# marcopesavento/Super-resolution-3D-Human-Shape-from-a-Single-Low-Resolution-Image

Hardware: AMD Instinct MI355X
Metric: occupancy queries/sec (dense 512^3 reconstruction: encoder + query sweep + 2x marching cubes) (higher is better)
Workload: dtype bf16

## Files before the change

super-resolution-3d-human-shape-from-a-single-low-resolution-image_amd/csrc/surs_api.cpp:

```cpp
#include "surs_common.h"

extern "C" int surs_abi_version(void) { return SURS_ABI_VERSION; }

extern "C" const char *surs_last_error(void) { return surs::err_buf(); }

extern "C" int surs_device_info(int *cu_count, char *arch_out) {
    int dev = 0;
    SURS_HIP_CHECK(hipGetDevice(&dev));
    hipDeviceProp_t prop;
    SURS_HIP_CHECK(hipGetDeviceProperties(&prop, dev));
    if (cu_count) *cu_count = prop.multiProcessorCount;
    if (arch_out) {
        strncpy(arch_out, prop.gcnArchName, 31);
        arch_out[31] = 0;
    }
    return 0;
}

#include <atomic>
#include <cstdlib>
#include <mutex>

namespace {
struct OptionRow {
    const char *name, *env;
    int def;
    char env_first;
    int env_value;
    const char *what;
};
const OptionRow kOptions[surs::OPT_COUNT] = {
    {"split_parts", "SURS_SPLIT", 2, 'b', 3, "operand parts of the fp32-grade GEMMs: 2 (f16 x 2) or 3 (bf16 x 3; env: bf16x3)"},
    {"grid_f32_columns", "SURS_GRID_F32", 1, 'g', 0, "0 (env: gemm): the fp32 sweep on the per-point layer kernels"},
    {"grid_kernel", "SURS_GRID_KERNEL", 0, 0, 0, "reduced-precision column kernel: 0 (default 12), 3, 10, 12"},
    {"grid_f32_kernel", "SURS_GRID_F32_KERNEL", 0, 0, 0, "fp32-grade column kernel: 0 (default 11), 5, 11"},
    {"r_parts", "SURS_R_PARTS", 1, 0, 0, "1: the bf16 sweep's R vectors from one f16 part; 0: the sweep's split"},
    {"grid_f32_passes", "SURS_GRID_F32_PASSES", 2, 0, 0, "passes of the fp32-grade column kernel per batch: 2 (lr, then hr) or 1"},
    {"bicubic_block", "SURS_BICUBIC_BLOCK", 1, 0, 0, "0: bicubic x2 with statistics one output per item (A/B; same bits)"},
    {"mc_emit_reclassify", "SURS_MC_EMIT_RECLASSIFY", 0, 0, 0, "1: marching cubes' emit pass classifies again (tests)"},
    {"point_runs_speculate", "SURS_POINT_RUNS_SPECULATE", 1, 0, 0, "0: surs_query_points_columns reads the run count before it launches"},
    {"conv_trace", "SURS_CONV_TRACE", 0, 0, 0, "diagnostic builds (-DSURS_CONV_TRACE): print the 3x3 kernel's phase stamps"},
    {"v3_trace", "SURS_V3_TRACE", 0, 0, 0, "diagnostic builds (-DSURS_V3_TRACE): print the column kernels' stamps"},
    {"conv_tall_min_wg", "SURS_CONV_TALL_MIN_WG", 256, 0, 0, "workgroups from which a stride-1 3x3 convolution takes the 8-row tile instead of 4 rows (0: never; same bits)"},
    {"conv_wide_min_wg", "SURS_CONV_WIDE_MIN_WG", 512, 0, 0, "workgroups (of 64 channels) from which such a launch takes 8 rows x 64 channels (part of the bits: another order of sums; 0: never)"},
    {"mc_ring", "SURS_MC_RING", 258, 0, 0, "planes of marching cubes' edge -> vertex-id ring = layers per chunk of a one-piece extraction + 1 (66: round 5's)"},
    {"rvec_small", "SURS_RVEC_SMALL", 1, 0, 0, "0: the affine part's GEMM of batches of <= 1024 columns on the 256 x 256-tile kernel (A/B; same bits)"},
};
std::atomic<int> g_option[surs::OPT_COUNT];
std::once_flag g_option_once;
void import_environment() {
    for (int i = 0; i < surs::OPT_COUNT; ++i) {
        const OptionRow &r = kOptions[i];
        int v = r.def;
        if (const char *e = getenv(r.env)) {
            if (r.env_first) v = (e[0] == r.env_first) ? r.env_value : r.def;
            else if (e[0]) v = atoi(e);
        }
        g_option[i].store(v, std::memory_order_relaxed);
    }
}
int find_option(const char *name) {
    if (!name) return -1;
    for (int i = 0; i < surs::OPT_COUNT; ++i)
        if (!strcmp(name, kOptions[i].name) || !strcmp(name, kOptions[i].env)) return i;
    return -1;
}
}

int surs::option(surs::Opt id) {
    std::call_once(g_option_once, import_environment);
    return g_option[id].load(std::memory_order_relaxed);
}

extern "C" int surs_set_option(const char *name, int value) {
    const int i = find_option(name);
    SURS_REQUIRE(i >= 0, "unknown option '%s' (surs_option_name(i) lists them)", name ? name : "(null)");
    std::call_once(g_option_once, import_environment);
    g_option[i].store(value, std::memory_order_relaxed);
    return 0;
}

extern "C" int surs_get_option(const char *name, int *value) {
    const int i = find_option(name);
    SURS_REQUIRE(i >= 0 && value, "unknown option '%s'", name ? name : "(null)");
    *value = surs::option((surs::Opt)i);
    return 0;
}

extern "C" const char *surs_option_name(int index) { return (index >= 0 && index < surs::OPT_COUNT) ? kOptions[index].name : nullptr; }
extern "C" const char *surs_option_help(int index) { return (index >= 0 && index < surs::OPT_COUNT) ? kOptions[index].what : nullptr; }
```

super-resolution-3d-human-shape-from-a-single-low-resolution-image_amd/csrc/surs_common.h:

```cpp
#pragma once
#include <hip/hip_runtime.h>

#include <cstdarg>
#include <cstdio>
#include <cstring>

#include "../../include/surs.h"

namespace surs {

inline char *err_buf() {
    static thread_local char buf[512] = "";
    return buf;
}

inline int fail(int code, const char *fmt, ...) {
    va_list ap;
    va_start(ap, fmt);
    vsnprintf(err_buf(), 512, fmt, ap);
    va_end(ap);
    return code;
}

#define SURS_HIP_CHECK(expr)                                                                     \
    do {                                                                                         \
        hipError_t e_ = (expr);                                                                  \
        if (e_ != hipSuccess)                                                                    \
            return surs::fail(SURS_E_HIP, "%s:%d %s -> %s", __FILE__, __LINE__, #expr, hipGetErrorString(e_)); \
    } while (0)

#define SURS_LAUNCH_CHECK() SURS_HIP_CHECK(hipGetLastError())

#define SURS_REQUIRE(cond, ...)                                   \
    do {                                                          \
        if (!(cond)) return surs::fail(SURS_E_INVALID, __VA_ARGS__); \
    } while (0)

#ifndef SURS_ABL_NO_ISA_PINS
#define SURS_ISA_PIN(v) asm volatile("" : "+v"(v))
#else
#define SURS_ISA_PIN(v) do { } while (0)
#endif

enum Opt {
    OPT_SPLIT_PARTS, OPT_GRID_F32_COLUMNS, OPT_GRID_KERNEL, OPT_GRID_F32_KERNEL, OPT_R_PARTS,
    OPT_GRID_F32_PASSES, OPT_BICUBIC_BLOCK, OPT_MC_EMIT_RECLASSIFY, OPT_POINT_RUNS_SPECULATE, OPT_CONV_TRACE,
    OPT_V3_TRACE, OPT_CONV_TALL_MIN_WG, OPT_CONV_WIDE_MIN_WG, OPT_MC_RING, OPT_RVEC_SMALL, OPT_COUNT
};
int option(Opt id);

inline hipStream_t as_stream(void *s) { return reinterpret_cast<hipStream_t>(s); }

constexpr int ceil_div(long long a, long long b) { return (int)((a + b - 1) / b); }

struct DeviceOnce {
    unsigned long long mask = 0;
    bool first() {
        int dev = 0;
        if (hipGetDevice(&dev) != hipSuccess || dev < 0 || dev >= 64) return true;
        const unsigned long long bit = 1ull << dev;
        const unsigned long long old = __atomic_fetch_or(&mask, bit, __ATOMIC_ACQ_REL);
        return !(old & bit);
    }
};
inline size_t align_up(size_t v, size_t a) { return (v + a - 1) / a * a; }

}
```

super-resolution-3d-human-shape-from-a-single-low-resolution-image_amd/csrc/surs_gemm.inc:

```
__device__ __forceinline__ bool gemm_block_tile(int mblocks, int nblocks, int &mb, int &nb) {
    const unsigned total = (unsigned)mblocks * (unsigned)nblocks, per = gridDim.x >> 3;
    const unsigned logical = (blockIdx.x & 7u) * per + (blockIdx.x >> 3);
    mb = (int)(logical % (unsigned)mblocks);
    nb = (int)(logical / (unsigned)mblocks);
    return logical < total;
}

static inline unsigned gemm_grid(int mblocks, long long nblocks) {
    const long long total = (long long)mblocks * nblocks;
    return (unsigned)(((total + 7) / 8) * 8);
}

struct SplitSeg {
    const unsigned short *base;
    long long part;
    int ktiles;
};

constexpr int G3_STAGES = 3;
constexpr int g3_stage_bytes(int bm, int np_ = 3) { return np_ * ((bm / 32) + 8) * 1024; }
constexpr int g3_lds_bytes(int bm, int np_ = 3) { return G3_STAGES * g3_stage_bytes(bm, np_); }

template <int NP> struct SplitKind;
template <> struct SplitKind<1> {
// ... 263 lines not shown
    const unsigned short *xp = a.g[m] + ((size_t)n0 + li) * 16 + kh * 8;
    const long long g_part = a.g_part[m];
    f32x16 acc[2];
#pragma unroll
    for (int j = 0; j < 2; ++j)
#pragma unroll
        for (int q = 0; q < 16; ++q) acc[j][q] = 0.0f;
    vec8 wf[PF][NP], xf[PF][2][NP];
    auto fetch = [&](int kt, int s) {
#pragma unroll
        for (int p = 0; p < NP; ++p) {
            wf[s][p] = *reinterpret_cast<const vec8 *>(wp + (size_t)kt * D2 * 16 + p * w_part);
#pragma unroll
            for (int j = 0; j < 2; ++j) xf[s][j][p] = *reinterpret_cast<const vec8 *>(xp + ((size_t)kt * npm + 32 * j) * 16 + p * g_part);
        }
    };
#pragma unroll
    for (int s = 0; s < PF; ++s) fetch(s, s);
    for (int k0 = 0; k0 < KT; k0 += PF) {
#pragma unroll
        for (int s = 0; s < PF; ++s) {
            vec8 w_[NP], x_[2][NP];
#pragma unroll
            for (int p = 0; p < NP; ++p) {
                w_[p] = wf[s][p];
                x_[0][p] = xf[s][0][p];
                x_[1][p] = xf[s][1][p];
            }
            if (k0 + PF + s < KT) fetch(k0 + PF + s, s);
#pragma unroll
            for (int t = 0; t < NP; ++t)
#pragma unroll
                for (int j = 0; j < 2; ++j) acc[j] = SK::mfma(x_[j][t], w_[NP - 1 - t], acc[j]);
            if (NP == 3) {
#pragma unroll
                for (int j = 0; j < 2; ++j) acc[j] = SK::mfma(x_[j][0], w_[1], acc[j]);
#pragma unroll
                for (int j = 0; j < 2; ++j) acc[j] = SK::mfma(x_[j][1], w_[0], acc[j]);
            }
            if (NP >= 2) {
#pragma unroll
                for (int j = 0; j < 2; ++j) acc[j] = SK::mfma(x_[j][0], w_[0], acc[j]);
            }
        }
    }
    float *out = a.r[m];
#pragma unroll
    for (int j = 0; j < 2; ++j)
#pragma unroll
        for (int gq = 0; gq < 4; ++gq)
#pragma unroll
            for (int r = 0; r < 4; ++r) out[(n0 + 32 * j + 4 * kh + 8 * gq + r) * D2 + m0 + li] = acc[j][4 * gq + r] + 0.0f;
}
```

super-resolution-3d-human-shape-from-a-single-low-resolution-image_amd/csrc/surs_query.hip:

```cpp
#include <hip/hip_runtime.h>

#include <cstdlib>
#include <map>
#include <mutex>
#include <type_traits>
#include <utility>
#include <vector>

#include "surs_common.h"
#include "surs_mlp_generic.h"
#include "surs_mlp_layout.h"

namespace surs {

typedef float f32x16 __attribute__((ext_vector_type(16)));
typedef float f32x4 __attribute__((ext_vector_type(4)));
typedef unsigned u32x4 __attribute__((ext_vector_type(4)));
typedef unsigned u32x2 __attribute__((ext_vector_type(2)));
typedef float f32x2 __attribute__((ext_vector_type(2)));

struct PointSource {
    int mode;
    const float *pts;
    const long long *idx;
// ... 66 lines not shown
    pix[1] = (long long)cy0 * W + cx1;
    pix[2] = (long long)cy1 * W + cx0;
    pix[3] = (long long)cy1 * W + cx1;
}

__device__ __forceinline__ float tap_sum(const float (&t)[4], const float (&w)[4]) {
    float a = 0.0f;
    a += t[0] * w[0];
    a += t[1] * w[1];
    a += t[2] * w[2];
    a += t[3] * w[3];
    return a;
}

typedef __bf16 bf16x8_t __attribute__((ext_vector_type(8)));
typedef unsigned short u16x8_t __attribute__((ext_vector_type(8)));

__device__ __forceinline__ void split3_bf16(float x, unsigned short &a, unsigned short &b, unsigned short &c) {
    const __bf16 ha = (__bf16)x;
    const float r1 = x - (float)ha;
    const __bf16 hb = (__bf16)r1;
    const float r2 = r1 - (float)hb;
    const __bf16 hc = (__bf16)r2;
    a = __builtin_bit_cast(unsigned short, ha);
    b = __builtin_bit_cast(unsigned short, hb);
    c = __builtin_bit_cast(unsigned short, hc);
}

#include "surs_gemm.inc"

template <int NP>
__global__ __launch_bounds__(256) void gather_kernel(PointSource src, long long n, const float *__restrict__ feat_lr,
                                                     int hl, int wl, const float *__restrict__ feat_hr, int hh,
                                                     int wh, float *__restrict__ F, long long ldf,
                                                     float *__restrict__ mask, float *__restrict__ zproj,
                                                     unsigned short *__restrict__ Fs, long long fs_part) {
    __shared__ float tile[64][65];
    __shared__ float sx[64], sy[64];
    const int tid = threadIdx.x, lane = tid & 63, wave = tid >> 6;
    const long long n0 = (long long)blockIdx.x * 64;
    const bool lead = blockIdx.y == 0;
    if (tid < 64) {
        long long t = n0 + tid;
        float X = 2.0f, Y = 2.0f;
        if (t < n) {
            float px, py, pz;
            make_point(src, t, px, py, pz);
            float Z;
            project_point(src, px, py, pz, X, Y, Z);
            const float in = in_image(X, Y);
            if (lead) {
                mask[t] = in;
                if (zproj) zproj[t] = Z;
                F[(long long)C_G * ldf + t] = Z * src.zmul / src.zdiv;
                F[(long long)(C_G + 1) * ldf + t] = 0.0f;
            }
            if (Fs && lead) {
                unsigned short zp[NP];
                SplitKind<NP>::split(Z * src.zmul / src.zdiv, zp);
#pragma unroll
                for (int p = 0; p < NP; ++p) {
                    u16x8_t v = {zp[p], 0, 0, 0, 0, 0, 0, 0}, z = {0, 0, 0, 0, 0, 0, 0, 0};
                    u16x8_t *dst = reinterpret_cast<u16x8_t *>(Fs + p * fs_part + ((long long)(C_G / 16) * ldf + t) * 16);
                    dst[0] = v;
                    dst[1] = z;
                }
            }
        }
        sx[tid] = X;
        sy[tid] = Y;
    }
    __syncthreads();
    for (int chunk = blockIdx.y; chunk < 5; chunk += gridDim.y) {
        const bool is_hr = chunk == 4;
        const float *feat = is_hr ? feat_hr : feat_lr;
        const int H = is_hr ? hh : hl, W = is_hr ? wh : wl, C = is_hr ? C_HR : C_LR;
        const int c0 = is_hr ? 0 : chunk * 64;
        for (int q0 = 0; q0 < 16; q0 += 8) {
            float t[8][4], w[8][4];
#pragma unroll
            for (int u4 = 0; u4 < 8; ++u4) {
                const int p = wave * 16 + q0 + u4;
                long long pix[4];
                bilinear_taps(sx[p], sy[p], H, W, pix, w[u4]);
                const long long ch = c0 + lane;
#pragma unroll
                for (int q = 0; q < 4; ++q) t[u4][q] = feat[pix[q] * C + ch];
            }
#pragma unroll
            for (int u4 = 0; u4 < 8; ++u4) tile[lane][wave * 16 + q0 + u4] = tap_sum(t[u4], w[u4]);
        }
        __syncthreads();
        const int cbase = is_hr ? C_LR : chunk * 64;
        for (int q = 0; q < 16; ++q) {
            const int ch = wave * 16 + q;
            if (n0 + lane < n) F[(long long)(cbase + ch) * ldf + n0 + lane] = tile[ch][lane];
        }
        if (Fs) {
#pragma unroll
            for (int it = 0; it < 2; ++it) {
                const int item = tid + 256 * it, p = item & 63, half = (item >> 6) & 1, ktl = item >> 7;
                u16x8_t q[NP];
#pragma unroll
                for (int j = 0; j < 8; ++j) {
                    unsigned short parts[NP];
                    SplitKind<NP>::split(tile[ktl * 16 + half * 8 + j][p], parts);
#pragma unroll
                    for (int k = 0; k < NP; ++k) q[k][j] = parts[k];
                }
                if (n0 + p < n) {
                    unsigned short *dst = Fs + ((long long)(cbase / 16 + ktl) * ldf + n0 + p) * 16 + half * 8;
#pragma unroll
                    for (int k = 0; k < NP; ++k) *reinterpret_cast<u16x8_t *>(dst + k * fs_part) = q[k];
                }
            }
        }
        __syncthreads();
    }
}

template <int NP>
__global__ __launch_bounds__(256) void mlp_last_kernel(const float *__restrict__ w4,
                                                       const float *__restrict__ Y3, const float *__restrict__ F,
                                                       long long ld, long long n, const float *__restrict__ mask,
                                                       float *__restrict__ pred, float *__restrict__ logit,
                                                       float *__restrict__ p_slot, unsigned short *__restrict__ Fs,
                                                       long long fs_part) {
    const long long t = (long long)blockIdx.x * 256 + threadIdx.x;
    if (t >= n) return;
    float acc = w4[D4 + C0PAD];
    for (int k = 0; k < D4; ++k) acc = fmaf(w4[k], Y3[(long long)k * ld + t], acc);
    for (int k = 0; k < C_G + 2; ++k) acc = fmaf(w4[D4 + k], F[(long long)k * ld + t], acc);
    const float p = mask[t] * (1.0f / (1.0f + expf(-acc)));
    pred[t] = p;
    if (logit) logit[t] = acc;
    if (p_slot) p_slot[t] = p;
    if (Fs) {
        unsigned short parts[NP];
        SplitKind<NP>::split(p, parts);
        unsigned short *dst = Fs + ((long long)(C_G / 16) * ld + t) * 16 + 1;
#pragma unroll
        for (int k = 0; k < NP; ++k) dst[k * fs_part] = parts[k];
    }
}

template <int NP>
__global__ __launch_bounds__(256) void patch_plr_kernel(const float *__restrict__ p_lr, long long ld, long long n, float *__restrict__ p_slot,
                                                        unsigned short *__restrict__ Fs, long long fs_part) {
    const long long t = (long long)blockIdx.x * 256 + threadIdx.x;
    if (t >= n) return;
// ... 55 lines not shown
    for (int k = 0; k < C_G + 2; ++k) acc = fmaf(w4[D4 + k], Fm[(long long)k * ld + t], acc);
    const float y = 1.0f / (1.0f + expf(-acc));
    if (logit) logit[t] = acc;
    for (int v = 0; v < nviews; ++v) {
        const float p = mask[(long long)v * ld + t] * y;
        pred[(long long)v * n + t] = p;
        if (p_slot) p_slot[(long long)v * f_view_stride + t] = p;
        if (Fs) {
            unsigned short parts[NP];
            SplitKind<NP>::split(p, parts);
            unsigned short *dst = Fs + (long long)v * NP * fs_part + ((long long)(C_G / 16) * ld + t) * 16 + 1;
#pragma unroll
            for (int k = 0; k < NP; ++k) dst[k * fs_part] = parts[k];
        }
    }
}

struct Fp32Workspace {
    float *F, *Y3, *mask;
    unsigned short *Fs, *Y0s, *Y1s, *Y2s;
    long long np;
};

static size_t fp32_ws_bytes(long long np) {
    return (size_t)np * ((C0PAD + D4 + 1) * sizeof(float) + (size_t)(C0PAD + D1 + D2 + D3) * 6) + 4096;
}

static Fp32Workspace carve_fp32(void *ws, long long np) {
    Fp32Workspace w;
    float *p = (float *)ws;
    w.np = np;
    w.F = p; p += (size_t)C0PAD * np;
    w.Y3 = p; p += (size_t)D4 * np;
    w.mask = p; p += np;
    unsigned short *q = (unsigned short *)p;
    w.Fs = q; q += (size_t)3 * C0PAD * np;
    w.Y0s = q; q += (size_t)3 * D1 * np;
    w.Y1s = q; q += (size_t)3 * D2 * np;
    w.Y2s = q;
    return w;
}

static int g_split_override = 0;
static thread_local int t_split_call = 0;
static int split_parts() {
    const int v = option(OPT_SPLIT_PARTS) == 3 ? 3 : 2;
    return t_split_call > 1 ? t_split_call : (g_split_override ? g_split_override : v);
}

template <int NP, int... More, class F> static void with_parts(int parts, F &&f) {
    if constexpr (sizeof...(More) == 0) f(std::integral_constant<int, NP>());
    else if (parts == NP) f(std::integral_constant<int, NP>());
    else with_parts<More...>(parts, f);
}

static int g3_set_attributes() {
    static DeviceOnce attr;
    if (attr.first()) {
        SURS_HIP_CHECK(hipFuncSetAttribute((const void *)gemm_x3g_kernel<8, 256, G3_SPLIT, 2>, hipFuncAttributeMaxDynamicSharedMemorySize, g3_lds_bytes(256, 2)));
        SURS_HIP_CHECK(hipFuncSetAttribute((const void *)gemm_x3g_kernel<8, 256, G3_F32, 2>, hipFuncAttributeMaxDynamicSharedMemorySize, g3_lds_bytes(256, 2)));
        SURS_HIP_CHECK(hipFuncSetAttribute((const void *)gemm_x3g_kernel<8, 128, G3_F32, 2>, hipFuncAttributeMaxDynamicSharedMemorySize, g3_lds_bytes(128, 2)));
        SURS_HIP_CHECK(hipFuncSetAttribute((const void *)gemm_x3g_kernel<8, 128, G3_F32_T, 2>, hipFuncAttributeMaxDynamicSharedMemorySize, g3_lds_bytes(128, 2)));
        SURS_HIP_CHECK(hipFuncSetAttribute((const void *)gemm_x3g_kernel<8, 256, G3_SPLIT>, hipFuncAttributeMaxDynamicSharedMemorySize, g3_lds_bytes(256)));
        SURS_HIP_CHECK(hipFuncSetAttribute((const void *)gemm_x3g_kernel<8, 256, G3_F32>, hipFuncAttributeMaxDynamicSharedMemorySize, g3_lds_bytes(256)));
        SURS_HIP_CHECK(hipFuncSetAttribute((const void *)gemm_x3g_kernel<8, 128, G3_F32>, hipFuncAttributeMaxDynamicSharedMemorySize, g3_lds_bytes(128)));
        SURS_HIP_CHECK(hipFuncSetAttribute((const void *)gemm_x3g_kernel<8, 128, G3_F32_T>, hipFuncAttributeMaxDynamicSharedMemorySize, g3_lds_bytes(128)));
        SURS_HIP_CHECK(hipFuncSetAttribute((const void *)gemm_x3g_kernel<8, 256, G3_F32_T, 2>, hipFuncAttributeMaxDynamicSharedMemorySize, g3_lds_bytes(256, 2)));
        SURS_HIP_CHECK(hipFuncSetAttribute((const void *)gemm_x3g_kernel<8, 256, G3_F32_T>, hipFuncAttributeMaxDynamicSharedMemorySize, g3_lds_bytes(256)));
        SURS_HIP_CHECK(hipFuncSetAttribute((const void *)gemm_x3g_kernel<8, 256, G3_F32_T, 1>, hipFuncAttributeMaxDynamicSharedMemorySize, g3_lds_bytes(256, 1)));
        SURS_HIP_CHECK(hipFuncSetAttribute((const void *)gemm_x3g_kernel<8, 256, G3_SPLIT, 1>, hipFuncAttributeMaxDynamicSharedMemorySize, g3_lds_bytes(256, 1)));
        SURS_HIP_CHECK(hipFuncSetAttribute((const void *)gemm_x3g_kernel<8, 256, G3_F32, 1>, hipFuncAttributeMaxDynamicSharedMemorySize, g3_lds_bytes(256, 1)));
        SURS_HIP_CHECK(hipFuncSetAttribute((const void *)gemm_x3g_kernel<8, 128, G3_F32, 1>, hipFuncAttributeMaxDynamicSharedMemorySize, g3_lds_bytes(128, 1)));
    }
    return 0;
}

static int launch_layer(hipStream_t st, int parts, int out, const void *W, int M, SplitSeg s1, SplitSeg s2, long long np, long long n,
                        const float *bias, float *Y, unsigned short *Ys) {
    SURS_REQUIRE(parts >= 1 && parts <= 3, "layer kernel: 1, 2 or 3 operand parts");
    SURS_REQUIRE(np % 256 == 0 && n % 256 == 0 && n <= np, "the layer kernel needs 256-point tiles");
    SURS_REQUIRE(M % 256 == 0 || (out != G3_SPLIT && M % 128 == 0), "layer kernel rows: a multiple of 256 (of 128 for an fp32 output)");
    SURS_REQUIRE(M % 256 == 0 || out != G3_F32_T || parts > 1, "no one-part layer kernel for a transposed output of 128-row tiles");
    int rc = g3_set_attributes();
    if (rc) return rc;
    const int K = 16 * (s1.ktiles + s2.ktiles), nb = (int)(n / 256);
    const long long ldy = out == G3_F32_T ? M : np;
    with_parts<1, 2, 3>(parts, [&](auto NP) {
        auto go = [&](auto BM, auto OUT) {
            hipLaunchKernelGGL((gemm_x3g_kernel<8, BM, OUT, NP>), dim3(gemm_grid(M / BM, nb)), dim3(512), g3_lds_bytes(BM, NP), st,
                               (const unsigned short *)W, M, K, s1, s2, np, bias, Y, ldy, Ys, (long long)M * np, nb);
        };
        using C256 = std::integral_constant<int, 256>;
        using C128 = std::integral_constant<int, 128>;
        if (out == G3_SPLIT) go(C256(), std::integral_constant<int, G3_SPLIT>());
        else if (out == G3_F32) {
            if (M % 256 == 0) go(C256(), std::integral_constant<int, G3_F32>());
            else go(C128(), std::integral_constant<int, G3_F32>());
        } else if (M % 256 == 0) go(C256(), std::integral_constant<int, G3_F32_T>());
        else if constexpr (NP > 1) go(C128(), std::integral_constant<int, G3_F32_T>());
    });
    SURS_LAUNCH_CHECK();
    return 0;
}

static int run_points_fp32(hipStream_t st, const PointSource &src, long long n, const float *feat_lr, int hl, int wl,
                           const float *feat_hr, int hh, int wh, const char *blob, const MlpBlobHeader &h,
// ... 58 lines not shown
    const float *colmask;
    const float *zvec;
    const char *core;
    const char *corex;
    const char *b1frag;
    const char *w1t;
    const char *w1tx;
    const float *rvec_lr, *rvec_hr;
    long long rld_lr, rld_hr;
    float zmid;
    unsigned *colctr;
    int phase;
    unsigned long long *kstat;
    float b1_inv_scale;
    float *vol_hr, *vol_lr;
    int ncols, rz;
    int zstride;
    const int *kcount;
    const unsigned short *klist;
    const int *colstart;
    const float *zpts;
    unsigned *ovf_count;
    int *ovf_list;
    const int *tile_list;
    const unsigned *tile_count;
    double z0, dz;
    float c22, c23;
    float zmul, zdiv;
};

__device__ __forceinline__ float lrelu01(float x) { return fmaxf(x, 0.01f * x); }

__device__ __forceinline__ unsigned opaque(unsigned v) {
    asm volatile("" : "+v"(v));
    return v;
}
__device__ __forceinline__ unsigned fresh_lane() {
    unsigned v;
    asm volatile("v_mbcnt_lo_u32_b32 %0, -1, 0\n\tv_mbcnt_hi_u32_b32 %0, -1, %0" : "=v"(v));
    return v;
}

#include "surs_grid_v3.inc"
#include "surs_grid_v5.inc"
#include "surs_grid_restated.inc"
#include "surs_grid_v10.inc"
#include "surs_grid_v12.inc"
#include "surs_grid_v11.inc"

template <int NP>
__global__ __launch_bounds__(256) void colsum_prepare_kernel(const float *__restrict__ cc, const float *__restrict__ zvec, int ncp,
                                                             float zmid, unsigned short *__restrict__ g_lr, long long part_lr,
                                                             unsigned short *__restrict__ g_hr, long long part_hr) {
    typedef SplitKind<NP> SK;
    __shared__ __attribute__((aligned(16))) unsigned stage[64][20][8];
    const int tid = threadIdx.x, lane = tid & 63, wave = tid >> 6;
    const int col0 = blockIdx.x * 4, col = col0 + wave;
    const int c16 = lane;
    const float *row = cc + (size_t)col * CC_PAD + 16 * c16;
    unsigned o[5][NP][8];
    {
        float a0l[16], a0h[16], wzl[16], wzh[16], wph[16];
#pragma unroll
        for (int j = 0; j < 16; j += 4) {
            const f32x4 t0 = *reinterpret_cast<const f32x4 *>(row + j), t1 = *reinterpret_cast<const f32x4 *>(row + CC_A0_HR + j);
            const f32x4 t2 = *reinterpret_cast<const f32x4 *>(zvec + ZV_W0Z_LR + 16 * c16 + j);
            const f32x4 t3 = *reinterpret_cast<const f32x4 *>(zvec + ZV_W0Z_HR + 16 * c16 + j);
            const f32x4 t4 = *reinterpret_cast<const f32x4 *>(zvec + ZV_W0P_HR + 16 * c16 + j);
#pragma unroll
            for (int e = 0; e < 4; ++e) {
                a0l[j + e] = t0[e]; a0h[j + e] = t1[e]; wzl[j + e] = t2[e]; wzh[j + e] = t3[e]; wph[j + e] = t4[e];
            }
        }
#pragma unroll
        for (int j = 0; j < 16; ++j) {
            const float gl = fmaf(zmid, wzl[j], a0l[j]) > 0.0f ? 1.0f : 0.01f;
            const float gh = fmaf(0.5f, wph[j], fmaf(zmid, wzh[j], a0h[j])) > 0.0f ? 1.0f : 0.01f;
            const float val[5] = {gl * a0l[j], gl * wzl[j], gh * a0h[j], gh * wzh[j], gh * wph[j]};
#pragma unroll
            for (int v = 0; v < 5; ++v) {
                unsigned short p[NP];
                SK::split(val[v], p);
#pragma unroll
                for (int q = 0; q < NP; ++q) {
                    if (j & 1) o[v][q][j >> 1] |= (unsigned)p[q] << 16;
                    else o[v][q][j >> 1] = p[q];
                }
            }
        }
    }
    const long long np_lr = 2LL * ncp, np_hr = 3LL * ncp;
#pragma unroll
    for (int q = 0; q < NP; ++q) {
        if (q) __syncthreads();
#pragma unroll
        for (int v = 0; v < 5; ++v) {
            const int slot = v < 2 ? 2 * wave + v : 8 + 3 * wave + (v - 2);
            *reinterpret_cast<u32x4 *>(&stage[c16][slot][0]) = u32x4{o[v][q][0], o[v][q][1], o[v][q][2], o[v][q][3]};
            *reinterpret_cast<u32x4 *>(&stage[c16][slot][4]) = u32x4{o[v][q][4], o[v][q][5], o[v][q][6], o[v][q][7]};
        }
        __syncthreads();
#pragma unroll
        for (int k = 0; k < 4; ++k) {
            const int item = tid + 256 * k, r = item >> 4, pc = item & 15;
            const u32x4 w = *reinterpret_cast<const u32x4 *>(&stage[r][0][0] + 4 * pc);
            *reinterpret_cast<u32x4 *>(g_lr + q * part_lr + ((long long)r * np_lr + 2LL * col0) * 16 + 8 * pc) = w;
        }
#pragma unroll
        for (int k = 0; k < 6; ++k) {
            const int item = tid + 256 * k, r = item / 24, pc = item - 24 * r;
            const u32x4 w = *reinterpret_cast<const u32x4 *>(&stage[r][8][0] + 4 * pc);
            *reinterpret_cast<u32x4 *>(g_hr + q * part_hr + ((long long)r * np_hr + 3LL * col0) * 16 + 8 * pc) = w;
        }
    }
}

}

using namespace surs;

static int zero_pad_rows(hipStream_t st, const Fp32Workspace &w) {
    SURS_HIP_CHECK(hipMemsetAsync(w.F + (size_t)(C_G + 2) * w.np, 0, (size_t)(C0PAD - C_G - 2) * w.np * sizeof(float), st));
    return 0;
}

#ifndef SURS_DEFAULT_GRID_KERNEL
#define SURS_DEFAULT_GRID_KERNEL 12
#endif
#ifndef SURS_DEFAULT_GRID_F32_KERNEL
#define SURS_DEFAULT_GRID_F32_KERNEL 11
#endif
static int g_grid_kernel_override = 0;
static bool grid_kernel_known(int v) { return v == 0 || v == 3 || v == 10 || v == 12 || v == 5 || v == 11; }
extern "C" int surs_set_grid_kernel(int version) {
    SURS_REQUIRE(grid_kernel_known(version),
// ... 280 lines not shown
    }
    if (tile_mlps) *tile_mlps = g_prof.tiles;
    if (ksteps) *ksteps = (double)v;
    return 0;
}

static const long long GRID_BATCH = 65536;
#ifndef SURS_COL_BATCH
#define SURS_COL_BATCH 32768
#endif
static const long long COL_BATCH = SURS_COL_BATCH;

static size_t col_base_bytes(long long ncb) {
    return (size_t)ncb * (C0PAD + CC_PAD + 1) * sizeof(float) + (size_t)ncb * C0PAD * 6 + 4096;
}
static size_t col_v7_image_bytes(long long ncb) { return (size_t)ncb * 5 * D1 * 6; }
static size_t col_v7_bytes(long long ncb) { return col_v7_image_bytes(ncb) + (size_t)ncb * 5 * D2 * 4 + D2 * 4 + 256; }
static size_t col_ws_bytes(long long ncb) { return col_base_bytes(ncb) + col_v7_bytes(ncb); }

extern "C" size_t surs_query_grid_workspace_bytes(int ry, int rz, int dtype) {
    (void)ry; (void)rz;
    const size_t col = col_ws_bytes(COL_BATCH);
    if (dtype == SURS_F32 || dtype == SURS_F32_GEMM) {
        const size_t gen = fp32_ws_bytes(GRID_BATCH);
        return gen > col ? gen : col;
    }
    return col;
}

static bool grid_f32_use_columns() { return option(OPT_GRID_F32_COLUMNS) != 0; }

static int grid_set_attributes() {
    static DeviceOnce attr;
    if (!attr.first()) return 0;
    SURS_HIP_CHECK(hipFuncSetAttribute((const void *)grid_mlp_kernel_v3<SURS_BF16>, hipFuncAttributeMaxDynamicSharedMemorySize, GRID3_LDS_BYTES));
    SURS_HIP_CHECK(hipFuncSetAttribute((const void *)grid_mlp_kernel_v3<SURS_F16>, hipFuncAttributeMaxDynamicSharedMemorySize, GRID3_LDS_BYTES));
    SURS_HIP_CHECK(hipFuncSetAttribute((const void *)grid_mlp_kernel_v5, hipFuncAttributeMaxDynamicSharedMemorySize, GRID5_LDS_BYTES));
    SURS_HIP_CHECK(hipFuncSetAttribute((const void *)grid_mlp_kernel_v11, hipFuncAttributeMaxDynamicSharedMemorySize, GRID11_LDS_BYTES));
    SURS_HIP_CHECK(hipFuncSetAttribute((const void *)grid_mlp_kernel_v10<SURS_BF16>, hipFuncAttributeMaxDynamicSharedMemorySize, GRID10_LDS_BYTES));
    SURS_HIP_CHECK(hipFuncSetAttribute((const void *)grid_mlp_kernel_v10<SURS_F16>, hipFuncAttributeMaxDynamicSharedMemorySize, GRID10_LDS_BYTES));
    SURS_HIP_CHECK(hipFuncSetAttribute((const void *)grid_mlp_kernel_v12<SURS_BF16>, hipFuncAttributeMaxDynamicSharedMemorySize, GRID12_LDS_BYTES));
    SURS_HIP_CHECK(hipFuncSetAttribute((const void *)grid_mlp_kernel_v12<SURS_F16>, hipFuncAttributeMaxDynamicSharedMemorySize, GRID12_LDS_BYTES));
    return 0;
}

static int column_constants(hipStream_t st, const PointSource &src, long long nc, long long ncp, const float *feat_lr, int hl, int wl,
                            const float *feat_hr, int hh, int wh, const char *blob, const MlpBlobHeader &h, float *F, float *CC,
                            float *cmask) {
    const int parts = split_parts();
    unsigned short *Fs = (unsigned short *)(cmask + COL_BATCH);
    const long long fs_part = (long long)C0PAD * COL_BATCH;
    const dim3 gg((unsigned)ceil_div(nc, 64), nc <= 4096 ? 5u : 1u);
    with_parts<2, 3>(parts, [&](auto NP) {
        hipLaunchKernelGGL(gather_kernel<NP>, gg, dim3(256), 0, st, src, nc, feat_lr, hl, wl, feat_hr, hh, wh, F, COL_BATCH, cmask,
                           (float *)nullptr, Fs, fs_part);
    });
    SURS_LAUNCH_CHECK();
    const SplitSeg f = {Fs, fs_part, C_G / 16}, none = {nullptr, 0, 0};
    return launch_layer(st, parts, G3_F32_T, blob + (parts == 2 ? h.wc2 : h.wc3), CC_PAD, f, none, COL_BATCH, ncp,
                        (const float *)(blob + h.bc), CC, nullptr);
}

__global__ __launch_bounds__(256) void probe_count_kernel(const float *__restrict__ cc, const float *__restrict__ zvec, int rz, int tile,
                                                          double z0, double dz, float c22, float c23, float zmul, float zdiv, float zmid,
                                                          unsigned long long *__restrict__ out) {
    const int tid = threadIdx.x;
    const float *row = cc + (size_t)blockIdx.x * CC_PAD;
    const f32x4 al = *reinterpret_cast<const f32x4 *>(row + CC_A0_LR + 4 * tid), ah = *reinterpret_cast<const f32x4 *>(row + CC_A0_HR + 4 * tid);
    const f32x4 zl = *reinterpret_cast<const f32x4 *>(zvec + ZV_W0Z_LR + 4 * tid), zh = *reinterpret_cast<const f32x4 *>(zvec + ZV_W0Z_HR + 4 * tid);
    const f32x4 ph = *reinterpret_cast<const f32x4 *>(zvec + ZV_W0P_HR + 4 * tid);
    auto zf_of = [&](int k) {
        const double zt = dz * (double)k;
        const float zw = (float)(zt + z0);
        const float Z = c23 + c22 * zw;
        return Z * zmul / zdiv;
    };
    unsigned nl = 0, nh = 0;
    for (int k0 = 0; k0 < rz; k0 += tile) {
        const float e0 = zf_of(k0), e1 = zf_of(k0 + tile - 1);
        const float zlo = fminf(e0, e1), zhi = fmaxf(e0, e1);
#pragma unroll
        for (int i = 0; i < 4; ++i) {
            {
                const float xm = fmaf(zmid, zl[i], al[i]);
                const float t0 = zl[i] * zlo, t1 = zl[i] * zhi;
                const float mn = al[i] + fminf(t0, t1), mx = al[i] + fmaxf(t0, t1);
                nl += ((xm > 0.0f) ? (mn > 0.0f) : (mx <= 0.0f)) ? 0u : 1u;
            }
            {
                const float xm = fmaf(0.5f, ph[i], fmaf(zmid, zh[i], ah[i]));
                const float t0 = zh[i] * zlo, t1 = zh[i] * zhi;
                const float mn = ah[i] + fminf(t0, t1) + fminf(0.0f, ph[i]), mx = ah[i] + fmaxf(t0, t1) + fmaxf(0.0f, ph[i]);
                nh += ((xm > 0.0f) ? (mn > 0.0f) : (mx <= 0.0f)) ? 0u : 1u;
            }
        }
    }
#pragma unroll
    for (int d = 32; d >= 1; d >>= 1) {
        nl += __shfl_xor(nl, d);
        nh += __shfl_xor(nh, d);
    }
    if ((tid & 63) == 0) {
        atomicAdd(out, (unsigned long long)nl);
        atomicAdd(out + 1, (unsigned long long)nh);
    }
}

static int query_grid_impl(int i0, int i1, int ry, int rz, const double *mat, const float *calib, float zmul,
// ... 64 lines not shown
static int device_cus() {
    int dev = 0;
    hipDeviceProp_t prop;
    if (hipGetDevice(&dev) == hipSuccess && hipGetDeviceProperties(&prop, dev) == hipSuccess) return prop.multiProcessorCount;
    return 256;
}

static int run_column_batch(const ColumnSweep &cs, const PointSource &src, long long nc, int items, int zstride,
                            const int *kcount, const unsigned short *klist, float *vol_hr, float *vol_lr, bool trace_this) {
    hipStream_t st = cs.st;
    const char *blob = cs.blob;
    const MlpBlobHeader &h = cs.h;
    const int dtype = cs.dtype, kver = cs.kver, kver32 = cs.kver32;
    const bool restated = cs.restated;
    const double *mat = cs.mat;
    const float *calib = cs.calib;
    void *workspace = cs.workspace;
    float *F = (float *)workspace;
    float *CC = F + (size_t)C0PAD * COL_BATCH;
    float *cmask = CC + (size_t)CC_PAD * COL_BATCH;
    int rc = 0;
    const long long ncp = (long long)ceil_div(nc, 256) * 256;
    const int parts = split_parts();
    if ((rc = column_constants(st, src, nc, ncp, cs.feat_lr, cs.hl, cs.wl, cs.feat_hr, cs.hh, cs.wh, blob, h, F, CC, cmask))) return rc;
    GridArgs a;
    a.cc = CC;
    a.colmask = cmask;
    a.zvec = (const float *)(blob + h.zvec);
    a.core = blob + h.core;
    a.corex = blob + h.corex;
    a.b1frag = blob + h.b1frag;
    a.b1_inv_scale = 1.0f / (dtype == SURS_F16 ? B1FRAG_SCALE_F16 : B1FRAG_SCALE_BF16);
    a.w1t = blob + h.w1t;
    a.w1tx = blob + h.w1tx;
    a.rvec_lr = a.rvec_hr = nullptr;
    a.rld_lr = a.rld_hr = 0;
    a.colctr = nullptr;
    a.phase = 0;
    a.zmid = 0.0f;
    a.zstride = zstride;
    a.kcount = kcount;
    a.klist = klist;
    a.ovf_count = nullptr;
    a.ovf_list = nullptr;
    a.tile_list = cs.run_tiles;
    a.tile_count = cs.run_ntiles;
    a.colstart = cs.run_colstart;
    a.zpts = cs.run_z;
    if (restated) {
        char *v7 = (char *)workspace + col_base_bytes(COL_BATCH);
        unsigned short *g_lr = (unsigned short *)v7, *g_hr = g_lr + (size_t)COL_BATCH * 2 * D1 * 3;
        float *r_lr = (float *)(v7 + col_v7_image_bytes(COL_BATCH)), *r_hr = r_lr + (size_t)COL_BATCH * 2 * D2;
        float *zero_bias = r_hr + (size_t)COL_BATCH * 3 * D2;
        SURS_HIP_CHECK(hipMemsetAsync(zero_bias, 0, D2 * 4 + 256, st));
        a.colctr = (unsigned *)(zero_bias + D2);
        {
            const float zw = cs.run_z ? 0.0f : (float)(mat[10] * (double)cs.kmid + mat[11]);
            a.zmid = (calib[11] + calib[10] * zw) * cs.zmul / cs.zdiv;
        }
        const long long part_lr = 2LL * ncp * D1, part_hr = 3LL * ncp * D1;
        const dim3 pg((unsigned)(ncp / 4));
        const int r_parts_env = option(OPT_R_PARTS);
        const int rparts = (dtype == SURS_BF16 && r_parts_env == 1) ? 1 : parts;
        with_parts<1, 2, 3>(rparts, [&](auto NP) {
            hipLaunchKernelGGL(colsum_prepare_kernel<NP>, pg, dim3(256), 0, st, CC, (const float *)(blob + h.zvec), (int)ncp, a.zmid,
                               g_lr, part_lr, g_hr, part_hr);
        });
        SURS_LAUNCH_CHECK();
        if (ncp <= 1024 && option(OPT_RVEC_SMALL)) {
            RvecSmallArgs ra;
            for (int m = 0; m < 2; ++m) {
                const int nvec = m ? 3 : 2;
                ra.w[m] = (const unsigned short *)(blob + (rparts == 3 ? h.wt3[m][1] : h.wt2[m][1]));
                ra.g[m] = m ? g_hr : g_lr;
                ra.g_part[m] = m ? part_hr : part_lr;
                ra.npm[m] = (long long)nvec * ncp;
                ra.r[m] = m ? r_hr : r_lr;
            }
            ra.wgs0 = (int)(ra.npm[0] / 64) * 4;
            const unsigned wgs = (unsigned)(ra.wgs0 + (ra.npm[1] / 64) * 4);
            with_parts<1, 2, 3>(rparts, [&](auto NP) { hipLaunchKernelGGL(rvec_small_kernel<NP>, dim3(wgs), dim3(256), 0, st, ra); });
            SURS_LAUNCH_CHECK();
        } else {
            const SplitSeg none = {nullptr, 0, 0};
            for (int m = 0; m < 2; ++m) {
                const long long npm = (m ? 3LL : 2LL) * ncp;
                const SplitSeg g = {m ? g_hr : g_lr, m ? part_hr : part_lr, D1 / 16};
                if ((rc = launch_layer(st, rparts, G3_F32_T, blob + (rparts == 3 ? h.wt3[m][1] : h.wt2[m][1]), D2, g, none, npm, npm,
                                       zero_bias, m ? r_hr : r_lr, nullptr)))
                    return rc;
            }
        }
        a.rvec_lr = r_lr;
        a.rvec_hr = r_hr;
        a.rld_lr = a.rld_hr = 0;
    }
    a.vol_hr = vol_hr;
    a.vol_lr = vol_lr;
    a.ncols = (int)nc;
    a.rz = items;
    a.z0 = mat ? mat[11] : 0.0;
    a.dz = mat ? mat[10] : 0.0;
    a.c22 = calib[10];
    a.c23 = calib[11];
    a.zmul = cs.zmul;
    a.zdiv = cs.zdiv;
    const long long nwork = cs.run_tiles ? cs.run_ntiles_host : nc;
    const unsigned grid = (unsigned)((nwork < cs.cus) ? nwork : cs.cus);
    hipEvent_t e0 = nullptr, e1 = nullptr;
    bool prof;
    a.kstat = nullptr;
    {
        std::lock_guard<std::mutex> lock(g_prof.mu);
        prof = g_prof.on && !kcount;
        if (prof && restated) {
            int dev = 0;
            SURS_HIP_CHECK(hipGetDevice(&dev));
            unsigned long long *&ctr = g_prof.kstat[dev];
            if (!ctr) {
                SURS_HIP_CHECK(hipMalloc((void **)&ctr, sizeof(unsigned long long)));
                SURS_HIP_CHECK(hipMemset(ctr, 0, sizeof(unsigned long long)));
            }
            a.kstat = ctr;
            g_prof.tiles += 2.0 * (double)nc * (dtype == SURS_F32 ? (items + 63) / 64 : (items + 127) / 128);
        }
    }
    if (prof) {
        SURS_HIP_CHECK(hipEventCreate(&e0));
        SURS_HIP_CHECK(hipEventCreate(&e1));
        SURS_HIP_CHECK(hipEventRecord(e0, st));
    }
    if (dtype == SURS_F32) {
        if (kver32 == 11) {
            const int passes_env = option(OPT_GRID_F32_PASSES);
            const bool two = passes_env == 2 && items % 64 == 0 && !cs.run_tiles;
            for (int ph = two ? 1 : 0; ph <= (two ? 2 : 0); ++ph) {
// ... 734 lines not shown
```

Before: 1.116 billion.

## Fuse column-batch R-vector prep into one GEMM kernel and skip fp32 F writes

Adds rvec_columns_kernel, which builds the gate-scaled split operands from the per-column coefficients directly in LDS and runs the R-vector GEMM in the same pass. This replaces colsum_prepare, two GEMM launches and a memset for batches above 1024 columns. The kernel also zeroes the column counters itself. Separately, the gather kernel no longer writes the fp32 F tensor when this path is on, because only the split Fs is consumed. This removes launches and an intermediate round trip through global memory, at the cost of a bespoke, hand-pipelined kernel that uses large LDS (up to 96 KB) and may cut occupancy.

```diff
diff --git a/super-resolution-3d-human-shape-from-a-single-low-resolution-image_amd/csrc/surs_api.cpp b/super-resolution-3d-human-shape-from-a-single-low-resolution-image_amd/csrc/surs_api.cpp
--- a/super-resolution-3d-human-shape-from-a-single-low-resolution-image_amd/csrc/surs_api.cpp
+++ b/super-resolution-3d-human-shape-from-a-single-low-resolution-image_amd/csrc/surs_api.cpp
@@ -45,6 +45,7 @@
     {"conv_wide_min_wg", "SURS_CONV_WIDE_MIN_WG", 512, 0, 0, "workgroups (of 64 channels) from which such a launch takes 8 rows x 64 channels (part of the bits: another order of sums; 0: never)"},
     {"mc_ring", "SURS_MC_RING", 258, 0, 0, "planes of marching cubes' edge -> vertex-id ring = layers per chunk of a one-piece extraction + 1 (66: round 5's)"},
     {"rvec_small", "SURS_RVEC_SMALL", 1, 0, 0, "0: the affine part's GEMM of batches of <= 1024 columns on the 256 x 256-tile kernel (A/B; same bits)"},
+    {"batch_prep", "SURS_BATCH_PREP", 1, 0, 0, "0: a column batch's R vectors by colsum_prepare + two GEMMs + memset, the gather's fp32 F written (A/B; same bits)"},
 };
 std::atomic<int> g_option[surs::OPT_COUNT];
 std::once_flag g_option_once;
diff --git a/super-resolution-3d-human-shape-from-a-single-low-resolution-image_amd/csrc/surs_common.h b/super-resolution-3d-human-shape-from-a-single-low-resolution-image_amd/csrc/surs_common.h
--- a/super-resolution-3d-human-shape-from-a-single-low-resolution-image_amd/csrc/surs_common.h
+++ b/super-resolution-3d-human-shape-from-a-single-low-resolution-image_amd/csrc/surs_common.h
@@ -45,7 +45,7 @@
 enum Opt {
     OPT_SPLIT_PARTS, OPT_GRID_F32_COLUMNS, OPT_GRID_KERNEL, OPT_GRID_F32_KERNEL, OPT_R_PARTS,
     OPT_GRID_F32_PASSES, OPT_BICUBIC_BLOCK, OPT_MC_EMIT_RECLASSIFY, OPT_POINT_RUNS_SPECULATE, OPT_CONV_TRACE,
-    OPT_V3_TRACE, OPT_CONV_TALL_MIN_WG, OPT_CONV_WIDE_MIN_WG, OPT_MC_RING, OPT_RVEC_SMALL, OPT_COUNT
+    OPT_V3_TRACE, OPT_CONV_TALL_MIN_WG, OPT_CONV_WIDE_MIN_WG, OPT_MC_RING, OPT_RVEC_SMALL, OPT_BATCH_PREP, OPT_COUNT
 };
 int option(Opt id);
 
diff --git a/super-resolution-3d-human-shape-from-a-single-low-resolution-image_amd/csrc/surs_gemm.inc b/super-resolution-3d-human-shape-from-a-single-low-resolution-image_amd/csrc/surs_gemm.inc
--- a/super-resolution-3d-human-shape-from-a-single-low-resolution-image_amd/csrc/surs_gemm.inc
+++ b/super-resolution-3d-human-shape-from-a-single-low-resolution-image_amd/csrc/surs_gemm.inc
@@ -339,3 +339,175 @@
 #pragma unroll
             for (int r = 0; r < 4; ++r) out[(n0 + 32 * j + 4 * kh + 8 * gq + r) * D2 + m0 + li] = acc[j][4 * gq + r] + 0.0f;
 }
+
+__device__ __forceinline__ float gscale_lr(float zmid, float w0z, float a0) { return fmaf(zmid, w0z, a0) > 0.0f ? 1.0f : 0.01f; }
+__device__ __forceinline__ float gscale_hr(float zmid, float w0z, float w0p, float a0) {
+    return fmaf(0.5f, w0p, fmaf(zmid, w0z, a0)) > 0.0f ? 1.0f : 0.01f;
+}
+template <int NP> __device__ __forceinline__ void gscaled_split(float g, float v, unsigned short (&p)[NP]) { SplitKind<NP>::split(g * v, p); }
+
+struct RvecColumnsArgs {
+    const unsigned short *w[2];
+    const float *cc;
+    const float *zvec;
+    float *r[2];
+    unsigned *counters;
+    float zmid;
+    int ncp;
+};
+constexpr int rvc_lds_bytes(int np_) { return 2 * np_ * 16384; }
+
+template <int NP, bool HR, int V>
+__device__ __forceinline__ void rvec_columns_tile(const RvecColumnsArgs &a, int cb, int mb, unsigned char *smem) {
+    typedef SplitKind<NP> SK;
+    typedef typename SK::vec8 vec8;
+    typedef unsigned u32x2 __attribute__((ext_vector_type(2)));
+    constexpr int KT = D1 / 16, UN = 4;
+    constexpr int RA = NP == 1 ? 4 : (NP == 2 ? 2 : 1), RZ = NP == 3 ? 1 : 2, RW = NP == 1 ? 2 : 1;
+    constexpr int STAGE = NP * 16384, PTS = NP * 8192, NVEC = HR ? 3 : 2;
+    static_assert(KT % UN == 0 && UN % RA == 0 && UN % RZ == 0 && UN % RW == 0, "register rings turn inside the unrolled steps");
+    const int tid = threadIdx.x, lane = tid & 63, wave = tid >> 6;
+    const int wm = wave >> 2, wn = wave & 3, kh = lane >> 5, li = lane & 31;
+    const int n0 = cb * 256, m0 = mb * 256;
+    const int q = tid & 3, c0 = tid >> 2;
+    const float zmid = a.zmid;
+    const float *ap = a.cc + (size_t)(n0 + c0) * CC_PAD + (HR ? CC_A0_HR : CC_A0_LR) + 4 * q;
+    const float *zp = a.zvec + (HR ? ZV_W0Z_HR : ZV_W0Z_LR) + 4 * q;
+    const float *pp = a.zvec + ZV_W0P_HR + 4 * q;
+    const unsigned short *wp = a.w[HR ? 1 : 0] + (size_t)m0 * 16 + tid * 8;
+    const int pdst = PTS + (c0 >> 5) * 1024 + ((q >> 1) * 32 + (c0 & 31)) * 16 + (q & 1) * 8;
+
+    f32x4 ra[RA][2], rz[RZ][HR ? 2 : 1];
+    u32x4 rw[RW][NP];
+    auto load_a = [&](int kt) {
+        const int kc = kt < KT ? kt : KT - 1;
+#pragma unroll
+        for (int i = 0; i < 2; ++i) ra[kt % RA][i] = *reinterpret_cast<const f32x4 *>(ap + (size_t)i * 128 * CC_PAD + 16 * kc);
+    };
+    auto load_z = [&](int kt) {
+        const int kc = kt < KT ? kt : KT - 1;
+        rz[kt % RZ][0] = *reinterpret_cast<const f32x4 *>(zp + 16 * kc);
+        if constexpr (HR) rz[kt % RZ][1] = *reinterpret_cast<const f32x4 *>(pp + 16 * kc);
+    };
+    auto load_w = [&](int kt) {
+        const int kc = kt < KT ? kt : KT - 1;
+#pragma unroll
+        for (int p = 0; p < NP; ++p) rw[kt % RW][p] = *reinterpret_cast<const u32x4 *>(wp + (size_t)kc * D2 * 16 + (size_t)p * D1 * D2);
+    };
+    auto build = [&](int kt) {
+        unsigned char *buf = smem + (kt & 1) * STAGE;
+#pragma unroll
+        for (int p = 0; p < NP; ++p) *reinterpret_cast<u32x4 *>(buf + p * 8192 + tid * 16) = rw[kt % RW][p];
+        const f32x4 wz = rz[kt % RZ][0];
+        f32x4 wpv = wz;
+        if constexpr (HR) wpv = rz[kt % RZ][1];
+#pragma unroll
+        for (int i = 0; i < 2; ++i) {
+            const f32x4 a0 = ra[kt % RA][i];
+            unsigned short h[4][NP];
+#pragma unroll
+            for (int e = 0; e < 4; ++e) {
+                const float g = HR ? gscale_hr(zmid, wz[e], wpv[e], a0[e]) : gscale_lr(zmid, wz[e], a0[e]);
+                const float x = V == 0 ? a0[e] : (V == 1 ? wz[e] : wpv[e]);
+                gscaled_split<NP>(g, x, h[e]);
+            }
+#pragma unroll
+            for (int p = 0; p < NP; ++p) {
+                const u32x2 o = {(unsigned)h[0][p] | ((unsigned)h[1][p] << 16), (unsigned)h[2][p] | ((unsigned)h[3][p] << 16)};
+                *reinterpret_cast<u32x2 *>(buf + pdst + p * 8192 + i * 4096) = o;
+            }
+        }
+    };
+
+    f32x16 acc[4][2];
+#pragma unroll
+    for (int i = 0; i < 4; ++i)
+#pragma unroll
+        for (int j = 0; j < 2; ++j)
+#pragma unroll
+            for (int r = 0; r < 16; ++r) acc[i][j][r] = 0.0f;
+    const int a_off = wm * 4096 + lane * 16, b_off = PTS + wn * 2048 + lane * 16;
+    auto products = [&](int kt) {
+        const unsigned char *buf = smem + (kt & 1) * STAGE;
+        vec8 af[4][NP], bf[2][NP];
+#pragma unroll
+        for (int p = 0; p < NP; ++p) {
+#pragma unroll
+            for (int i = 0; i < 4; ++i) af[i][p] = *reinterpret_cast<const vec8 *>(buf + a_off + p * 8192 + i * 1024);
+#pragma unroll
+            for (int j = 0; j < 2; ++j) bf[j][p] = *reinterpret_cast<const vec8 *>(buf + b_off + p * 8192 + j * 1024);
+        }
+        auto mm = [&](int pa, int pb) {
+#pragma unroll
+            for (int i = 0; i < 4; ++i)
+#pragma unroll
+                for (int j = 0; j < 2; ++j) acc[i][j] = SK::mfma(bf[j][pb], af[i][pa], acc[i][j]);
+        };
+#pragma unroll
+        for (int t = 0; t < NP; ++t) mm(NP - 1 - t, t);
+        if constexpr (NP == 3) {
+            mm(1, 0);
+            mm(0, 1);
+        }
+        if constexpr (NP > 1) mm(0, 0);
+    };
+
+    auto step_barrier = [&]() { asm volatile("s_waitcnt lgkmcnt(0)\n\ts_barrier" ::: "memory"); };
+#pragma unroll
+    for (int s = 0; s < RW; ++s) load_w(s);
+#pragma unroll
+    for (int s = 0; s < RZ; ++s) load_z(s);
+#pragma unroll
+    for (int s = 0; s < RA; ++s) load_a(s);
+    build(0);
+    __builtin_amdgcn_sched_barrier(0);
+    load_w(RW);
+    load_z(RZ);
+    load_a(RA);
+    __builtin_amdgcn_sched_barrier(0);
+    step_barrier();
+    for (int k0 = 0; k0 < KT; k0 += UN) {
+#pragma unroll
+        for (int s = 0; s < UN; ++s) {
+            const int kt = k0 + s;
+            build(kt + 1);
+            products(kt);
+            __builtin_amdgcn_sched_barrier(0);
+            load_w(kt + 1 + RW);
+            load_z(kt + 1 + RZ);
+            load_a(kt + 1 + RA);
+            __builtin_amdgcn_sched_barrier(0);
+            step_barrier();
+        }
+    }
+
+    float *out = a.r[HR ? 1 : 0];
+#pragma unroll
+    for (int i = 0; i < 4; ++i)
+#pragma unroll
+        for (int j = 0; j < 2; ++j) {
+            const int row = m0 + wm * 128 + i * 32 + li;
+            const int col = n0 + wn * 64 + j * 32 + 4 * kh;
+#pragma unroll
+            for (int g = 0; g < 4; ++g)
+#pragma unroll
+                for (int r = 0; r < 4; ++r) out[((size_t)(col + 8 * g + r) * NVEC + V) * D2 + row] = acc[i][j][4 * g + r] + 0.0f;
+        }
+}
+
+template <int NP>
+__global__ __launch_bounds__(512) void rvec_columns_kernel(RvecColumnsArgs a) {
+    extern __shared__ __attribute__((aligned(16))) unsigned char rvc_smem[];
+    if (blockIdx.x == 0 && threadIdx.x < 64) a.counters[threadIdx.x] = 0u;
+    const unsigned total = (unsigned)(a.ncp / 256) * 10u, per = gridDim.x >> 3;
+    const unsigned logical = (blockIdx.x & 7u) * per + (blockIdx.x >> 3);
+    if (logical >= total) return;
+    const int cb = (int)(logical / 10u), s = (int)(logical % 10u);
+    switch (s >> 1) {
+    case 0: rvec_columns_tile<NP, false, 0>(a, cb, s & 1, rvc_smem); break;
+    case 1: rvec_columns_tile<NP, false, 1>(a, cb, s & 1, rvc_smem); break;
+    case 2: rvec_columns_tile<NP, true, 0>(a, cb, s & 1, rvc_smem); break;
+    case 3: rvec_columns_tile<NP, true, 1>(a, cb, s & 1, rvc_smem); break;
+    default: rvec_columns_tile<NP, true, 2>(a, cb, s & 1, rvc_smem); break;
+    }
+}
diff --git a/super-resolution-3d-human-shape-from-a-single-low-resolution-image_amd/csrc/surs_query.hip b/super-resolution-3d-human-shape-from-a-single-low-resolution-image_amd/csrc/surs_query.hip
--- a/super-resolution-3d-human-shape-from-a-single-low-resolution-image_amd/csrc/surs_query.hip
+++ b/super-resolution-3d-human-shape-from-a-single-low-resolution-image_amd/csrc/surs_query.hip
@@ -142,8 +142,10 @@
             if (lead) {
                 mask[t] = in;
                 if (zproj) zproj[t] = Z;
-                F[(long long)C_G * ldf + t] = Z * src.zmul / src.zdiv;
-                F[(long long)(C_G + 1) * ldf + t] = 0.0f;
+                if (F) {
+                    F[(long long)C_G * ldf + t] = Z * src.zmul / src.zdiv;
+                    F[(long long)(C_G + 1) * ldf + t] = 0.0f;
+                }
             }
             if (Fs && lead) {
                 unsigned short zp[NP];
@@ -182,10 +184,11 @@
         }
         __syncthreads();
         const int cbase = is_hr ? C_LR : chunk * 64;
-        for (int q = 0; q < 16; ++q) {
-            const int ch = wave * 16 + q;
-            if (n0 + lane < n) F[(long long)(cbase + ch) * ldf + n0 + lane] = tile[ch][lane];
-        }
+        if (F)
+            for (int q = 0; q < 16; ++q) {
+                const int ch = wave * 16 + q;
+                if (n0 + lane < n) F[(long long)(cbase + ch) * ldf + n0 + lane] = tile[ch][lane];
+            }
         if (Fs) {
 #pragma unroll
             for (int it = 0; it < 2; ++it) {
@@ -347,6 +350,16 @@
     if constexpr (sizeof...(More) == 0) f(std::integral_constant<int, NP>());
     else if (parts == NP) f(std::integral_constant<int, NP>());
     else with_parts<More...>(parts, f);
+}
+
+static int rvc_set_attributes() {
+    static DeviceOnce attr;
+    if (attr.first()) {
+        SURS_HIP_CHECK(hipFuncSetAttribute((const void *)rvec_columns_kernel<1>, hipFuncAttributeMaxDynamicSharedMemorySize, rvc_lds_bytes(1)));
+        SURS_HIP_CHECK(hipFuncSetAttribute((const void *)rvec_columns_kernel<2>, hipFuncAttributeMaxDynamicSharedMemorySize, rvc_lds_bytes(2)));
+        SURS_HIP_CHECK(hipFuncSetAttribute((const void *)rvec_columns_kernel<3>, hipFuncAttributeMaxDynamicSharedMemorySize, rvc_lds_bytes(3)));
+    }
+    return 0;
 }
 
 static int g3_set_attributes() {
@@ -511,7 +524,6 @@
 __global__ __launch_bounds__(256) void colsum_prepare_kernel(const float *__restrict__ cc, const float *__restrict__ zvec, int ncp,
                                                              float zmid, unsigned short *__restrict__ g_lr, long long part_lr,
                                                              unsigned short *__restrict__ g_hr, long long part_hr) {
-    typedef SplitKind<NP> SK;
     __shared__ __attribute__((aligned(16))) unsigned stage[64][20][8];
     const int tid = threadIdx.x, lane = tid & 63, wave = tid >> 6;
     const int col0 = blockIdx.x * 4, col = col0 + wave;
@@ -533,13 +545,13 @@
         }
 #pragma unroll
         for (int j = 0; j < 16; ++j) {
-            const float gl = fmaf(zmid, wzl[j], a0l[j]) > 0.0f ? 1.0f : 0.01f;
-            const float gh = fmaf(0.5f, wph[j], fmaf(zmid, wzh[j], a0h[j])) > 0.0f ? 1.0f : 0.01f;
-            const float val[5] = {gl * a0l[j], gl * wzl[j], gh * a0h[j], gh * wzh[j], gh * wph[j]};
+            const float gl = gscale_lr(zmid, wzl[j], a0l[j]);
+            const float gh = gscale_hr(zmid, wzh[j], wph[j], a0h[j]);
+            const float gv[5] = {gl, gl, gh, gh, gh}, val[5] = {a0l[j], wzl[j], a0h[j], wzh[j], wph[j]};
 #pragma unroll
             for (int v = 0; v < 5; ++v) {
                 unsigned short p[NP];
-                SK::split(val[v], p);
+                gscaled_split<NP>(gv[v], val[v], p);
 #pragma unroll
                 for (int q = 0; q < NP; ++q) {
                     if (j & 1) o[v][q][j >> 1] |= (unsigned)p[q] << 16;
@@ -926,8 +938,8 @@
     const long long fs_part = (long long)C0PAD * COL_BATCH;
     const dim3 gg((unsigned)ceil_div(nc, 64), nc <= 4096 ? 5u : 1u);
     with_parts<2, 3>(parts, [&](auto NP) {
-        hipLaunchKernelGGL(gather_kernel<NP>, gg, dim3(256), 0, st, src, nc, feat_lr, hl, wl, feat_hr, hh, wh, F, COL_BATCH, cmask,
-                           (float *)nullptr, Fs, fs_part);
+        hipLaunchKernelGGL(gather_kernel<NP>, gg, dim3(256), 0, st, src, nc, feat_lr, hl, wl, feat_hr, hh, wh,
+                           option(OPT_BATCH_PREP) ? (float *)nullptr : F, COL_BATCH, cmask, (float *)nullptr, Fs, fs_part);
     });
     SURS_LAUNCH_CHECK();
     const SplitSeg f = {Fs, fs_part, C_G / 16}, none = {nullptr, 0, 0};
@@ -1098,7 +1110,6 @@
         unsigned short *g_lr = (unsigned short *)v7, *g_hr = g_lr + (size_t)COL_BATCH * 2 * D1 * 3;
         float *r_lr = (float *)(v7 + col_v7_image_bytes(COL_BATCH)), *r_hr = r_lr + (size_t)COL_BATCH * 2 * D2;
         float *zero_bias = r_hr + (size_t)COL_BATCH * 3 * D2;
-        SURS_HIP_CHECK(hipMemsetAsync(zero_bias, 0, D2 * 4 + 256, st));
         a.colctr = (unsigned *)(zero_bias + D2);
         {
             const float zw = cs.run_z ? 0.0f : (float)(mat[10] * (double)cs.kmid + mat[11]);
@@ -1108,12 +1119,33 @@
         const dim3 pg((unsigned)(ncp / 4));
         const int r_parts_env = option(OPT_R_PARTS);
         const int rparts = (dtype == SURS_BF16 && r_parts_env == 1) ? 1 : parts;
-        with_parts<1, 2, 3>(rparts, [&](auto NP) {
-            hipLaunchKernelGGL(colsum_prepare_kernel<NP>, pg, dim3(256), 0, st, CC, (const float *)(blob + h.zvec), (int)ncp, a.zmid,
-                               g_lr, part_lr, g_hr, part_hr);
-        });
-        SURS_LAUNCH_CHECK();
-        if (ncp <= 1024 && option(OPT_RVEC_SMALL)) {
+        const bool small = ncp <= 1024 && option(OPT_RVEC_SMALL);
+        const bool fused = !small && option(OPT_BATCH_PREP);
+        if (fused) {
+            if ((rc = rvc_set_attributes())) return rc;
+            RvecColumnsArgs ra;
+            for (int m = 0; m < 2; ++m) {
+                ra.w[m] = (const unsigned short *)(blob + (rparts == 3 ? h.wt3[m][1] : h.wt2[m][1]));
+                ra.r[m] = m ? r_hr : r_lr;
+            }
+            ra.cc = CC;
+            ra.zvec = (const float *)(blob + h.zvec);
+            ra.counters = a.colctr;
+            ra.zmid = a.zmid;
+            ra.ncp = (int)ncp;
+            with_parts<1, 2, 3>(rparts, [&](auto NP) {
+                hipLaunchKernelGGL(rvec_columns_kernel<NP>, dim3(gemm_grid(10, ncp / 256)), dim3(512), rvc_lds_bytes(NP), st, ra);
+            });
+            SURS_LAUNCH_CHECK();
+        } else {
+            SURS_HIP_CHECK(hipMemsetAsync(zero_bias, 0, D2 * 4 + 256, st));
+            with_parts<1, 2, 3>(rparts, [&](auto NP) {
+                hipLaunchKernelGGL(colsum_prepare_kernel<NP>, pg, dim3(256), 0, st, CC, (const float *)(blob + h.zvec), (int)ncp, a.zmid,
+                                   g_lr, part_lr, g_hr, part_hr);
+            });
+            SURS_LAUNCH_CHECK();
+        }
+        if (small) {
             RvecSmallArgs ra;
             for (int m = 0; m < 2; ++m) {
                 const int nvec = m ? 3 : 2;
@@ -1127,7 +1159,7 @@
             const unsigned wgs = (unsigned)(ra.wgs0 + (ra.npm[1] / 64) * 4);
             with_parts<1, 2, 3>(rparts, [&](auto NP) { hipLaunchKernelGGL(rvec_small_kernel<NP>, dim3(wgs), dim3(256), 0, st, ra); });
             SURS_LAUNCH_CHECK();
-        } else {
+        } else if (!fused) {
             const SplitSeg none = {nullptr, 0, 0};
             for (int m = 0; m < 2; ++m) {
                 const long long npm = (m ? 3LL : 2LL) * ncp;
```

Result: no change. 1.126 billion, median of 6 (+0.9%).
